# snakers4/mnasnet-pytorch

Measured on AMD Instinct MI355X. Metric: images/sec MNASNet-1.0 224^2 bf16 train step, higher is better.
Workload: dtype bf16

## Files before the change

include/mnas.h:

```cpp
#ifndef MNAS_H
#define MNAS_H
#include <stdint.h>

#ifdef __cplusplus
extern "C" {
#endif

#define MNAS_OK 0
#define MNAS_EINVAL 10001
#define MNAS_BN_ROWS 8

typedef struct MnasActIn {
    const void*  data;
    const float* scale;
    const float* shift;
} MnasActIn;

typedef struct MnasGradIn {
    const void*  g;
    const void*  y;
    const float* coef;
} MnasGradIn;

int mnas_version(void);
const char* mnas_arch(void);

typedef struct MnasConvGemm {
    int32_t mode;
    int32_t N, Hi, Wi, Ci;
    int32_t Ho, Wo, Co;
    int32_t kh, kw, stride, pad;
    int32_t nparts;
    int32_t reserved;
    MnasActIn  act;
    MnasGradIn grad;
    const void*  w;
    const float* bias;
    const void*  resid;
    void*        out;
    float*       stats;
    const void*  red_y;
    const float* red_bn;
    const float* gate;
} MnasConvGemm;
int mnas_conv_gemm_gate_ok(int N, int HW, int Ci, int Co);
int mnas_conv_gemm(const MnasConvGemm* a, void* stream);
int mnas_conv_gemm_tile_pixels(int M, int Co, int K);
int mnas_conv_gemm_parts(int mode, int M, int Ci, int Co, int taps);
int mnas_conv_img_parts(int mode, int N, int Hi, int Wi, int Ci, int Ho, int Wo, int Co, int k, int stride, int pad);
#define MNAS_ROUTE_PWX   0
#define MNAS_ROUTE_PWS   1
#define MNAS_ROUTE_PWF   2
#define MNAS_ROUTE_PWD   3
#define MNAS_ROUTE_C3R   4
#define MNAS_ROUTE_DIMG  5
#define MNAS_ROUTE_C3X   6
#define MNAS_ROUTE_IGEMM 7
int mnas_conv_gemm_route(const MnasConvGemm* a, int* out);

typedef struct MnasTconvDgrad {
    int32_t N, Ho, Wo, Co, Ci, nparts;
    const void* dy;
    const void* w;
    void* out;
    float* stats;
    const void* red_y;
    const float* red_bn;
} MnasTconvDgrad;
int mnas_tconv_dgrad(const MnasTconvDgrad* a, void* stream);
int mnas_tconv_supported(int Ho, int Wo, int Co, int Ci);
int mnas_tconv_parts(int N, int Ho, int Wo, int Co, int Ci);

typedef struct MnasConvWgrad {
    int32_t N, Hi, Wi, Ci;
    int32_t Ho, Wo, Co;
    int32_t kh, kw, stride, pad;
    int32_t nsplit;
    MnasActIn  x;
    MnasGradIn dy;
    float* partial;
} MnasConvWgrad;
int mnas_conv_wgrad(const MnasConvWgrad* a, void* stream);
int mnas_conv_wgrad_slabs(int Co, int Ci, int taps);

int mnas_wgrad_finalize(float* partial, int nsplit, int Co, int Ci, int taps,
                        float* grad, int accumulate, void* stream);

typedef struct MnasPwBwd {
    int32_t M, Ci, Co, nparts;
    MnasActIn  x;
    MnasGradIn dy;
    const void* w;
    const void* resid;
    void*  gin;
    float* wpartial;
    float* red_partial;
    const void*  red_y;
    const float* red_bn;
    const void*  w_fwd;
    const float* b_fwd;
    int32_t gin_masked;
    int32_t seg_px;
} MnasPwBwd;
int mnas_pw_bwd(const MnasPwBwd* a, void* stream);
int mnas_pw_bwd_supported(int Ci, int Co);
int mnas_pw_bwd_tile_pixels(int Ci, int Co);
int mnas_pw_bwd_slices(int Ci, int Co);
int mnas_pw_bwd_forms(int Ci, int Co);

typedef struct MnasDwFwd {
    int32_t N, H, W, C, k;
    int32_t nparts;
    MnasActIn in;
    const float* w;
    const float* bias;
    void*  out;
    float* stats;
    int32_t stride, reserved;
} MnasDwFwd;
int mnas_dw_fwd(const MnasDwFwd* a, void* stream);
int mnas_dw_geometry(int N, int H, int W, int C, int k, int which, int* out);
int mnas_dw_rows(int N, int H, int W, int C, int k, int nparts, int which);

typedef struct MnasDwBwd {
    int32_t N, H, W, C, k;
    int32_t nparts;
    MnasActIn  x;
    MnasGradIn dy;
    const float* w;
    void*  gin;
    float* wpartial;
    const float* red_bn;
    float* red_partial;
    int32_t phase;
    int32_t stride;
    int32_t g_masked, reserved;
} MnasDwBwd;
int mnas_dw_bwd(const MnasDwBwd* a, void* stream);
int mnas_dw_wgrad_finalize(float* wpartial, int nparts, int C, int k, float* grad, int accumulate,
                           void* stream);

typedef struct MnasStemFwd {
    int32_t N, H, W, Ho, Wo, Co;
    int32_t nparts;
    const float* x;
    const void*  w;
    const float* bias;
    void*  out;
    float* stats;
    const float* in_affine;
    int32_t in_u8, reserved;
} MnasStemFwd;
int mnas_stem_fwd(const MnasStemFwd* a, void* stream);
typedef struct MnasStemWgrad {
    int32_t N, H, W, Ho, Wo, Co;
    int32_t nparts;
    const float* x;
    MnasGradIn dy;
    float* partial;
    const float* in_affine;
    int32_t in_u8, reserved;
} MnasStemWgrad;
int mnas_stem_wgrad(const MnasStemWgrad* a, void* stream);
int mnas_stem_parts(int which, int N, int H, int W, int Co);
int mnas_stem_dgrad(const MnasGradIn* dy, const float* w, int N, int H, int W, int Ho, int Wo, int Co, const float* in_affine,
                    float* dx, void* stream);

int mnas_bn_fwd_finalize(const float* partial, int nparts, int C, double count,
                         const float* gamma, const float* beta,
                         float* running_mean, float* running_var, int64_t* num_batches_tracked,
                         float momentum, float eps, int training, float* bnbuf, void* stream);
int mnas_bn_bwd_reduce(const void* g, const void* y, const float* bnbuf, int64_t rows, int C,
                       int nparts, float* partial, void* stream);
int mnas_dy_materialize(const MnasGradIn* d, int64_t rows, int C, void* out_bf16, void* stream);
int mnas_bn_bwd_finalize(const float* partial, int nparts, int C, double count,
                         float* bnbuf, float* dgamma, float* dbeta, int accumulate, void* stream);

typedef struct MnasPostWgrad {
    float* partial;
    float* grad;
    int32_t nsplit, Co, Ci, taps, dw, level;
} MnasPostWgrad;
typedef struct MnasBwdPost {
    const float* bn_partial;
    float* bnbuf;
    float* dgamma;
    float* dbeta;
    double count;
    int32_t bn_nparts, bn_C;
    MnasPostWgrad w1, w2;
} MnasBwdPost;
int mnas_bwd_post(const MnasBwdPost* p, void* stream);

typedef struct MnasBnFrozenDesc {
    const float* gamma;
    const float* beta;
    const float* running_mean;
    const float* running_var;
    float*  bnbuf;
    int32_t C;
    float   eps;
} MnasBnFrozenDesc;
int mnas_bn_frozen_tables(const MnasBnFrozenDesc* descs, int n, void* stream);
int mnas_bn_bwd_finalize_frozen(const float* partial, int nparts, int C, const float* bnbuf, float* dgamma, float* dbeta,
                                float* dbias, int accumulate, void* stream);
typedef struct MnasBwdPostFrozen {
    const float* bn_partial;
    const float* bnbuf;
    float* dgamma;
    float* dbeta;
    double count;
// ... 284 lines not shown
```

mnasnet_pytorch_amd/_lib.py:

```python
from __future__ import annotations

import ctypes as C
import os

import torch

_HERE = os.path.dirname(os.path.abspath(__file__))
ABI_VERSION = 8
LIB_PATH = os.environ.get("MNAS_LIB_PATH") or os.path.join(_HERE, "csrc", "libmnas_hip.so")

c_void_p, c_int, c_float, c_double, c_int64 = C.c_void_p, C.c_int, C.c_float, C.c_double, C.c_int64


class MnasActIn(C.Structure):
    _fields_ = [("data", c_void_p), ("scale", c_void_p), ("shift", c_void_p)]


class MnasGradIn(C.Structure):
    _fields_ = [("g", c_void_p), ("y", c_void_p), ("coef", c_void_p)]


class MnasConvGemm(C.Structure):
    _fields_ = [("mode", C.c_int32), ("N", C.c_int32), ("Hi", C.c_int32), ("Wi", C.c_int32), ("Ci", C.c_int32),
                ("Ho", C.c_int32), ("Wo", C.c_int32), ("Co", C.c_int32), ("kh", C.c_int32), ("kw", C.c_int32),
# ... 160 lines not shown
    OP_BWD_POST: (("bn_nparts", "bn_C") + _post("w1") + _post("w2"), ("count",),
                  ("bn_partial", "bnbuf", "dgamma", "dbeta", "w1.partial", "w1.grad", "w2.partial", "w2.grad")),
    OP_BWD_POST_FROZEN: (("bn_nparts", "bn_C") + _post("w1") + _post("w2"), ("count",),
                         ("bn_partial", "bnbuf", "dgamma", "dbeta", "w1.partial", "w1.grad", "w2.partial", "w2.grad", "dbias")),
    OP_BN_BWD_FINALIZE_FROZEN: (("nparts", "C", "accumulate"), (), ("partial", "bnbuf", "dgamma", "dbeta", "dbias")),
    OP_BN_FROZEN_BATCH: (("n",), (), ("descs",)),
    OP_TCONV_DGRAD: (("N", "Ho", "Wo", "Co", "Ci", "nparts"), (), ("dy", "w", "out", "stats", "red_y", "red_bn")),
    OP_HEAD_LINEAR: (("N", "I", "O", "relu", "accumulate", "which"), (),
                     ("x", "w", "b", "y", "dz", "dw", "db", "dx", "relu_mask")),
    OP_SE_SCALE: (("N", "HW", "C"), (), _act("a") + ("u", "out")),
    OP_SE_BWD_REDUCE: (("N", "HW", "C"), (), ("gs",) + _act("a") + ("u", "du", "scratch")),
    OP_SE_BWD_APPLY: (("N", "HW", "C"), (), ("gs", "u", "dz", "out", "red_y", "red_bn", "red_partial")),
    OP_SE_GATE: (("N", "C"), (), ("u", "gate")),
    OP_SE_PROJ_FIN: (("N", "kseg", "Co", "Ci", "accumulate"), (), ("wpartial", "u", "w", "grad", "du")),
    OP_SE_FC_FWD: (("N", "E", "R"), (), ("z", "w1", "b1", "w2", "b2", "hb", "u", "gate")),
    OP_SE_FC_BWD: (("N", "E", "R", "accumulate"), (), ("du", "z", "hb", "w1", "w2", "dh", "dz", "dw1", "db1", "dw2", "db2")),
}
OP_STREAM_SLOT = 14
_SLOT = {}
_GROUP = {}
for _opc, _kinds in OP_SLOTS.items():
    _SLOT[_opc], _GROUP[_opc] = {}, {}
    for _kind, _names in zip("idp", _kinds):
        for _k, _name in enumerate(_names):
            if _name is None:
                continue
            if _name in _SLOT[_opc] or (_kind == "i" and _k >= OP_STREAM_SLOT):
                raise ValueError("OP_SLOTS[%d]: bad slot %s" % (_opc, _name))
            _SLOT[_opc][_name] = (_kind, _k)
            if "." in _name:
                _GROUP[_opc].setdefault(_name.split(".")[0], []).append(_name)


def slot(opcode, name):
    return _SLOT[opcode][name][1]


def set_op(o, opcode, stream=0, **fields):
    slots, oi, od, op = _SLOT[opcode], o.i, o.d, o.p
    o.opcode, oi[OP_STREAM_SLOT] = opcode, stream
    for name, v in fields.items():
        where = slots.get(name)
        if where is None:
            members = _GROUP[opcode].get(name)
            if members is None:
                raise TypeError("opcode %d: unknown slot %s" % (opcode, name))
            if hasattr(v, "_asdict"):
                v = [getattr(v, m.split(".")[1]) for m in members]
            elif hasattr(v, "act_ptrs"):
                v = v.act_ptrs()
            if len(v) != len(members) or any(m in fields for m in members):
                raise TypeError("opcode %d: group %s takes %d values, once" % (opcode, name, len(members)))
            set_op(o, opcode, stream, **dict(zip(members, v)))
            continue
        kind, k = where
        if kind == "i":
            oi[k] = v
        elif kind == "d":
            od[k] = v
        else:
            op[k] = (v if v is None or type(v) is int else v.data_ptr()) or None
    return o


def op_field(o, name):
    kind, k = _SLOT[o.opcode][name]
    return getattr(o, kind)[k]


def op_ints(o):
    return tuple(int(v) for v in o.i[:len(OP_SLOTS[o.opcode][0])])


class MnasHeadLinear(C.Structure):
    _fields_ = [("N", C.c_int32), ("I", C.c_int32), ("O", C.c_int32), ("relu", C.c_int32), ("accumulate", C.c_int32),
                ("drop_p", c_float), ("seed", C.c_uint64), ("x", c_void_p), ("w", c_void_p), ("b", c_void_p),
                ("y", c_void_p), ("dz", c_void_p), ("dw", c_void_p), ("db", c_void_p), ("dx", c_void_p),
                ("relu_mask", c_void_p)]


METERS_MAX_K, METERS_NUM_I64, METERS_NUM_F64 = 4, 14, 3


class MnasMeters(C.Structure):
    _fields_ = [("steps", c_int64), ("samples", c_int64), ("loss_samples", c_int64), ("nonfinite_steps", c_int64),
                ("correct", c_int64 * 4), ("last_n", c_int64), ("last_loss_n", c_int64), ("last_correct", c_int64 * 4),
                ("loss_sum", c_double), ("last_loss", c_double), ("last_loss_sum", c_double)]


MLABEL_NUM_I64, MLABEL_NUM_F64 = 16, 9


class MnasMultiLabelMeters(C.Structure):
    _fields_ = [(n, c_int64) for n in ("steps", "samples", "nonfinite_steps", "loss_n", "dice_n", "f1_n", "tp", "fp", "fn", "last_n",
                                       "last_loss_n", "last_dice_n", "last_f1_n", "last_tp", "last_fp", "last_fn")] + \
               [(n, c_double) for n in ("loss_sum", "dice_sum", "f1_sum", "last_loss", "last_dice", "last_f1", "last_loss_sum",
                                        "last_dice_sum", "last_f1_sum")]


GRADNORM_MAX_PARTS = 1024


class MnasGradStats(C.Structure):
    _fields_ = [("last_norm", c_float), ("last_coef", c_float), ("steps", c_int64), ("clipped_steps", c_int64),
                ("skipped_steps", c_int64)]


class MnasOptExtra(C.Structure):
    _fields_ = [("partial", c_void_p), ("nparts", C.c_int32), ("max_norm", c_float), ("skip_nonfinite", C.c_int32),
                ("ema", c_void_p), ("ema_decay", c_float), ("stats", c_void_p), ("update_stats", C.c_int32)]


SYMBOLS = {
    "mnas_conv_img_parts": (c_int, [c_int] * 11),
    "mnas_stem_parts": (c_int, [c_int, c_int, c_int, c_int, c_int]),
    "mnas_head_linear_fwd": (c_int, [C.POINTER(MnasHeadLinear), c_void_p]),
    "mnas_head_linear_bwd_w": (c_int, [C.POINTER(MnasHeadLinear), c_void_p]),
    "mnas_head_linear_bwd_x": (c_int, [C.POINTER(MnasHeadLinear), c_void_p]),
    "mnas_head_dropout_mask": (c_int, [c_void_p, c_int64, c_float, C.c_uint64, c_void_p]),
    "mnas_head_cross_entropy": (c_int, [c_void_p, c_void_p, c_int, c_int, c_int64, c_void_p, c_void_p, c_void_p, c_void_p,
                                        c_void_p]),
    "mnas_head_cross_entropy_metrics": (c_int, [c_void_p, c_void_p, c_int, c_int, c_int64, c_void_p, c_void_p, c_void_p, c_void_p,
                                                C.POINTER(c_int), c_int, c_void_p, c_void_p, c_void_p]),
    "mnas_head_metrics": (c_int, [c_void_p, c_void_p, c_int, c_int, C.POINTER(c_int), c_int, c_void_p, c_void_p, c_void_p,
                                  c_void_p]),
    "mnas_head_cross_entropy_soft": (c_int, [c_void_p, c_void_p, c_void_p, c_void_p, c_float, c_int, c_int, c_int64, c_void_p,
                                             c_void_p, c_void_p, c_void_p, C.POINTER(c_int), c_int, c_void_p, c_void_p, c_void_p]),
    "mnas_mlabel_scratch_bytes": (c_int64, [c_int]),
    "mnas_mlabel_bce": (c_int, [c_void_p, c_void_p, c_void_p, c_int, c_int, c_int, c_float, c_float, c_void_p, c_void_p, c_void_p,
                                c_void_p, c_int64, c_int64, c_int64, c_void_p]),
    "mnas_mlabel_metrics": (c_int, [c_void_p, c_void_p, c_int, c_int, c_void_p, c_void_p, c_void_p, c_int64, c_int64, c_int64,
                                    c_void_p]),
    "mnas_mlabel_hard_dice": (c_int, [c_void_p, c_void_p, c_int, c_int, c_float, c_int, c_void_p, c_void_p, c_void_p]),
    "mnas_se_scale": (c_int, [C.POINTER(MnasActIn), c_void_p, c_int, c_int, c_int, c_void_p, c_void_p]),
    "mnas_se_bwd_reduce": (c_int, [c_void_p, C.POINTER(MnasActIn), c_void_p, c_int, c_int, c_int, c_void_p, c_void_p, c_void_p]),
    "mnas_se_scratch_bytes": (c_int64, [c_int, c_int, c_int]),
    "mnas_se_bwd_apply": (c_int, [c_void_p, c_void_p, c_void_p, c_int, c_int, c_int, c_void_p, c_void_p, c_void_p, c_void_p, c_void_p]),
    "mnas_se_bwd_apply_cols": (c_int, [c_int, c_int, c_int]),
    "mnas_se_gate": (c_int, [c_void_p, c_int, c_int, c_void_p, c_void_p]),
    "mnas_se_proj_finalize": (c_int, [c_void_p, c_int, c_int, c_int, c_int, c_void_p, c_void_p, c_void_p, c_int, c_void_p, c_void_p]),
    "mnas_stem_dgrad": (c_int, [c_void_p, c_void_p] + [c_int] * 6 + [c_void_p] * 3),
    "mnas_se_fc_supported": (c_int, [c_int, c_int]),
    "mnas_se_fc_fwd": (c_int, [c_void_p] * 5 + [c_int] * 3 + [c_void_p] * 4),
    "mnas_se_fc_bwd": (c_int, [c_void_p] * 5 + [c_int] * 3 + [c_void_p] * 6 + [c_int, c_void_p]),
    "mnas_conv_gemm_gate_ok": (c_int, [c_int, c_int, c_int, c_int]),
    "mnas_graph_create": (c_int, [C.POINTER(MnasOp), c_int, C.POINTER(c_void_p), c_int, C.POINTER(c_void_p), C.POINTER(c_int)]),
    "mnas_graph_launch": (c_int, [c_void_p, c_void_p]),
    "mnas_graph_destroy": (c_int, [c_void_p]),
    "mnas_version": (c_int, []),
    "mnas_arch": (C.c_char_p, []),
    "mnas_workspace_bytes": (c_int64, [c_int, c_int, c_int, c_int]),
    "mnas_conv_gemm": (c_int, [C.POINTER(MnasConvGemm), c_void_p]),
    "mnas_conv_gemm_route": (c_int, [C.POINTER(MnasConvGemm), C.POINTER(c_int)]),
    "mnas_conv_gemm_tile_pixels": (c_int, [c_int, c_int, c_int]),
    "mnas_conv_gemm_parts": (c_int, [c_int, c_int, c_int, c_int, c_int]),
    "mnas_conv_wgrad": (c_int, [C.POINTER(MnasConvWgrad), c_void_p]),
    "mnas_conv_wgrad_slabs": (c_int, [c_int, c_int, c_int]),
    "mnas_wgrad_finalize": (c_int, [c_void_p, c_int, c_int, c_int, c_int, c_void_p, c_int, c_void_p]),
    "mnas_pw_bwd": (c_int, [C.POINTER(MnasPwBwd), c_void_p]),
    "mnas_pw_bwd_supported": (c_int, [c_int, c_int]),
    "mnas_pw_bwd_forms": (c_int, [c_int, c_int]),
    "mnas_pw_bwd_tile_pixels": (c_int, [c_int, c_int]),
    "mnas_pw_bwd_slices": (c_int, [c_int, c_int]),
    "mnas_dw_fwd": (c_int, [C.POINTER(MnasDwFwd), c_void_p]),
    "mnas_dw_bwd": (c_int, [C.POINTER(MnasDwBwd), c_void_p]),
    "mnas_dw_rows": (c_int, [c_int, c_int, c_int, c_int, c_int, c_int, c_int]),
    "mnas_dw_geometry": (c_int, [c_int, c_int, c_int, c_int, c_int, c_int, C.POINTER(c_int)]),
    "mnas_dw_wgrad_finalize": (c_int, [c_void_p, c_int, c_int, c_int, c_void_p, c_int, c_void_p]),
    "mnas_stem_fwd": (c_int, [C.POINTER(MnasStemFwd), c_void_p]),
    "mnas_stem_wgrad": (c_int, [C.POINTER(MnasStemWgrad), c_void_p]),
    "mnas_bn_fwd_finalize": (c_int, [c_void_p, c_int, c_int, c_double, c_void_p, c_void_p, c_void_p, c_void_p,
                                     c_void_p, c_float, c_float, c_int, c_void_p, c_void_p]),
    "mnas_bn_bwd_reduce": (c_int, [c_void_p, c_void_p, c_void_p, c_int64, c_int, c_int, c_void_p, c_void_p]),
    "mnas_tconv_dgrad": (c_int, [C.POINTER(MnasTconvDgrad), c_void_p]),
    "mnas_tconv_supported": (c_int, [c_int, c_int, c_int, c_int]),
    "mnas_tconv_parts": (c_int, [c_int, c_int, c_int, c_int, c_int]),
    "mnas_bwd_post": (c_int, [C.POINTER(MnasBwdPost), c_void_p]),
    "mnas_bwd_post_frozen": (c_int, [C.POINTER(MnasBwdPostFrozen), c_void_p]),
    "mnas_bn_bwd_finalize_frozen": (c_int, [c_void_p, c_int, c_int, c_void_p, c_void_p, c_void_p, c_void_p, c_int, c_void_p]),
    "mnas_bn_frozen_tables": (c_int, [c_void_p, c_int, c_void_p]),
    "mnas_dy_materialize": (c_int, [C.POINTER(MnasGradIn), c_int64, c_int, c_void_p, c_void_p]),
    "mnas_bn_bwd_finalize": (c_int, [c_void_p, c_int, c_int, c_double, c_void_p, c_void_p, c_void_p, c_int, c_void_p]),
    "mnas_add_act": (c_int, [C.POINTER(MnasActIn), C.POINTER(MnasActIn), c_int64, c_int, c_void_p, c_void_p, c_int,
                             c_void_p]),
    "mnas_pool_act": (c_int, [C.POINTER(MnasActIn), c_int, c_int, c_int, c_void_p, c_void_p]),
    "mnas_pool_bwd": (c_int, [c_void_p, c_int, c_int, c_int, c_void_p, c_void_p]),
    "mnas_nchw_f32_to_nhwc_bf16": (c_int, [c_void_p, c_void_p, c_int, c_int, c_int, c_void_p]),
    "mnas_pack_weights": (c_int, [c_void_p, c_int, c_int, c_int, c_int, c_int, c_void_p, c_void_p]),
    "mnas_pack_weights_batch": (c_int, [c_void_p, c_int, c_void_p]),
    "mnas_packed_bytes": (c_int64, [c_int, c_int, c_int, c_int, c_int]),
    "mnas_adam_step": (c_int, [c_void_p, c_void_p, c_void_p, c_void_p, c_int64, c_float, c_float, c_float, c_float,
                               c_float, c_int, c_float, c_void_p]),
    "mnas_rmsprop_step": (c_int, [c_void_p, c_void_p, c_void_p, c_void_p, c_int64, c_float, c_float, c_float, c_float, c_float,
                                  c_float, c_void_p]),
    "mnas_sgd_step": (c_int, [c_void_p, c_void_p, c_void_p, c_int64, c_float, c_float, c_float, c_float, c_int, c_int, c_float,
                              c_void_p]),
    "mnas_grad_sqnorm": (c_int, [c_void_p, c_int64, c_float, c_void_p, c_int, C.POINTER(c_int), c_void_p]),
    "mnas_adam_step_ex": (c_int, [c_void_p, c_void_p, c_void_p, c_void_p, c_int64, c_float, c_float, c_float, c_float,
                                  c_float, c_int, c_float, C.POINTER(MnasOptExtra), c_void_p]),
    "mnas_rmsprop_step_ex": (c_int, [c_void_p, c_void_p, c_void_p, c_void_p, c_int64, c_float, c_float, c_float, c_float, c_float,
                                     c_float, C.POINTER(MnasOptExtra), c_void_p]),
    "mnas_sgd_step_ex": (c_int, [c_void_p, c_void_p, c_void_p, c_int64, c_float, c_float, c_float, c_float, c_int, c_int, c_float,
                                 C.POINTER(MnasOptExtra), c_void_p]),
    "mnas_run_ops": (c_int, [C.POINTER(MnasOp), c_int, c_void_p, C.POINTER(c_int)]),
    "mnas_run_ops_multi": (c_int, [C.POINTER(MnasOp), c_int, C.POINTER(c_void_p), c_int, C.POINTER(c_int)]),
    "mnas_event_create": (c_int, [C.POINTER(c_void_p)]),
    "mnas_event_destroy": (c_int, [c_void_p]),
    "mnas_event_record": (c_int, [c_void_p, c_void_p]),
    "mnas_event_elapsed_ms": (c_int, [c_void_p, c_void_p, C.POINTER(c_float)]),
    "mnas_probe_copy": (c_int, [c_void_p, c_void_p, c_int64, c_void_p]),
    "mnas_probe_valu": (c_int, [c_void_p, c_int, c_int, c_void_p]),
    "mnas_probe_copy4": (c_int, [c_void_p, c_void_p, c_int64, c_int, c_void_p]),
    "mnas_probe_read": (c_int, [c_void_p, c_void_p, c_int64, c_int, c_void_p]),
    "mnas_probe_empty": (c_int, [c_int, c_int, c_void_p]),
    "mnas_img_xform_check": (c_int, [C.POINTER(MnasImgXform), c_int, c_int, c_int, c_int64]),
    "mnas_img_xform": (c_int, [c_void_p, c_int, c_int, c_int, c_void_p, c_int64, c_void_p, c_void_p]),
    "mnas_img_color_check": (c_int, [C.POINTER(MnasImgColor), c_int, c_int, c_int]),
    "mnas_img_color_workspace_bytes": (c_int64, [c_int, c_int, c_int]),
    "mnas_img_color": (c_int, [c_void_p, c_int, c_int, c_int, c_int, c_void_p, c_int, c_void_p, c_void_p, c_void_p]),
    "mnas_img_mix_check": (c_int, [C.POINTER(MnasImgMix), c_int, c_int, c_int]),
    "mnas_img_mix": (c_int, [c_void_p, c_int, c_int, c_int, c_void_p, c_void_p, c_void_p]),
}

_lib = None


def load():
    global _lib
    if _lib is not None:
        return _lib
    if not os.path.exists(LIB_PATH):
        raise RuntimeError(
            "libmnas_hip.so not built (%s): run `make -C mnasnet_pytorch_amd/csrc` or __graft_entry__.build(). "
            "There is no CPU / eager fallback for the MNASNet hot path." % LIB_PATH)
    lib = C.CDLL(LIB_PATH)
    for name, (res, args) in SYMBOLS.items():
        fn = getattr(lib, name)
        fn.restype = res
        fn.argtypes = args
    if lib.mnas_version() != ABI_VERSION:
        raise RuntimeError("libmnas_hip.so ABI version %d != %d (stale build: run make -C mnasnet_pytorch_amd/csrc)" % (lib.mnas_version(), ABI_VERSION))
    _lib = lib
    return lib


def check(rc, what="mnas call"):
    if rc != 0:
        raise RuntimeError("%s failed with code %d" % (what, rc))


def cur_stream():
    return torch.cuda.current_stream().cuda_stream


def ptr(t):
    return 0 if t is None else t.data_ptr()
```

mnasnet_pytorch_amd/csrc/mnas_gemm.hip:

```cpp
#include "mnas_common.h"

struct IgemmArgs {
    int M, Hi, Wi, Ci, Ho, Wo, Co;
    int kh, kw, stride, pad;
    int Ktot, Kpad, kch, taps, is_pw, co_pad16;
    int s2, Mc, tpc;
    MnasActIn act;
    MnasGradIn grad;
    const uint16_t* w;
    const float* bias;
    const void* resid;
    void* out;
    float* stats;
    const void* red_y;
    const float* red_bn;
    int nt;
    float rcp_hw, rcp_wo, rcp_ci;
    const float* gate;
};

template <int MODE, int NT, int PT, int KCH, bool PIPE, bool PAR2, bool GATE = false>
__global__ __launch_bounds__(256) void k_igemm(IgemmArgs a) {
    static_assert(!GATE || (MODE == 0 && !PAR2), "the gate is an act-on-load extension of the 1x1 forward");
    extern __shared__ __attribute__((aligned(16))) unsigned char smem[];
// ... 426 lines not shown
    if (a.s2) a.tpc = (a.Mc + 64 * PT - 1) / (64 * PT);
    const int ntiles = a.s2 ? 4 * a.tpc : (a.M + 64 * PT - 1) / (64 * PT);
    const int nkc = (a.Kpad + a.kch - 1) / a.kch;
    const int phases = nkc * ((ntiles + nparts - 1) / nparts);
    const bool s2 = a.taps > 1 && a.stride == 2;
    bool pipe;
    if (MODE == 0) pipe = phases >= 4 && !(s2 && PT == 2) && !(NT >= 6 && PT == 2);
    else pipe = phases >= 2 && nkc > 1 && !s2;
    if constexpr (PT == 1 && (NT == 2 || NT == 3 || NT == 4 || NT == 6)) {
        if (a.kch == 128) return launch_igemm_k<MODE, NT, PT, 128>(a, nparts, nblocks, pipe, stream);
    }
    return a.kch >= 64 ? launch_igemm_k<MODE, NT, PT, 64>(a, nparts, nblocks, pipe, stream)
                       : launch_igemm_k<MODE, NT, PT, 32>(a, nparts, nblocks, pipe, stream);
}

static void igemm_tiling(int Co, int Kpad, int M, int* nt_out, int* nblocks_out, int* pt_out) {
    const int tiles = (Co + 15) / 16;
    int best_nt = 1, best_waste = 1 << 30, best_blocks = 1 << 30;
    if (tiles <= 8) {
        static const int opts1[] = {1, 2, 3, 4, 6, 8};
        for (int nt : opts1) if (nt >= tiles) { best_nt = nt; best_blocks = 1; break; }
    } else {
        static const int opts_small_k[3] = {4, 3, 0}, opts_large_k[3] = {6, 4, 3};
        for (int nt : (Kpad >= 512 ? opts_large_k : opts_small_k)) {
            if (nt == 0) continue;
            const int blocks = (tiles + nt - 1) / nt;
            const int waste = blocks * nt - tiles;
            if (waste < best_waste || (waste == best_waste && blocks < best_blocks)) {
                best_nt = nt; best_waste = waste; best_blocks = blocks;
            }
        }
    }
    *nt_out = best_nt;
    *nblocks_out = best_blocks;
    *pt_out = ((int64_t)M * best_blocks >= (int64_t)128 * 1024) ? 2 : 1;
}

extern "C" int mnas_conv_gemm_tile_pixels(int M, int Co, int K) {
    if (M < 1 || Co < 1 || K < 1) return -1;
    int nt, nblocks, pt;
    igemm_tiling(Co, (K + 31) / 32 * 32, M, &nt, &nblocks, &pt);
    return 64 * pt;
}

extern "C" int mnas_conv_gemm_parts(int mode, int M, int Ci, int Co, int taps) {
    if (mode == 0 && taps == 1) {
        const int p = mnas_pwx_parts(M, Ci, Co);
        if (p > 0) return p;
    }
    if (taps == 1) {
        const int p = mnas_pws_parts(mode, M, Ci, Co);
        if (p > 0) return p;
    }
    if (mode == 0 && taps == 1 && mnas_pwf_enabled()) return mnas_pwf_parts(M, Ci, Co);
    if (mode == 1 && taps == 1 && mnas_pwd_enabled()) return mnas_pwd_parts(M, Ci, Co);
    return -1;
}

extern "C" int mnas_conv_gemm_gate_ok(int N, int HW, int Ci, int Co) {
    if (N < 1 || HW < 1 || (Ci & 7) || (Co & 7) || Ci < 8 || Co < 8) return 0;
    const int M = N * HW;
    if (mnas_pws_parts(0, M, Ci, Co) > 0) return mnas_pws_gate_ok(M, Ci, Co);
    int nt, nblocks, pt;
    igemm_tiling(Co, (Ci + 31) / 32 * 32, M, &nt, &nblocks, &pt);
    return (nt <= 3 && nblocks == 1 && !(pt == 1 && Ci >= 256) && HW >= 64 * pt) ? 1 : 0;
}

static int conv_gemm_plan(const MnasConvGemm* c, IgemmArgs* ap, int* nt_out, int* nblocks_out, int* pt_out) {
    if (!c || (c->mode != 0 && c->mode != 1)) return -MNAS_EINVAL;
    if ((c->Ci & 7) || (c->Co & 7) || c->nparts < 1 || c->nparts > 65535) return -MNAS_EINVAL;
    IgemmArgs& a = *ap;
    a.M = c->N * c->Ho * c->Wo;
    a.Hi = c->Hi; a.Wi = c->Wi; a.Ci = c->Ci; a.Ho = c->Ho; a.Wo = c->Wo; a.Co = c->Co;
    a.kh = c->kh; a.kw = c->kw; a.stride = c->stride; a.pad = c->pad;
    a.taps = c->kh * c->kw;
    a.Ktot = a.taps * c->Ci;
    a.Kpad = (a.Ktot + 31) / 32 * 32;
    a.kch = a.Kpad >= 64 ? 64 : 32;
    a.is_pw = (a.taps == 1 && c->stride == 1 && c->pad == 0) ? 1 : 0;
    a.co_pad16 = (c->Co + 15) / 16 * 16;
    a.act = c->act; a.grad = c->grad;
    a.w = (const uint16_t*)c->w; a.bias = c->bias; a.resid = c->resid; a.out = c->out; a.stats = c->stats;
    a.red_y = (c->mode == 1) ? c->red_y : nullptr; a.red_bn = c->red_bn;
    a.nt = (mnas_nt_mask() & (c->mode == 1 ? MNAS_NT_IGEMM_DGRAD : MNAS_NT_IGEMM_FWD)) ? 1 : 0;
    a.gate = c->gate;
    if (a.gate && (c->mode != 0 || !a.is_pw || !c->act.scale || c->resid)) return -MNAS_EINVAL;
    {
        const int s2f = (c->mode == 1 && c->kh == 3 && c->kw == 3 && c->stride == 2 && c->pad == 1 && !(c->Ho & 1) && !(c->Wo & 1));
        const int wd = s2f ? c->Wo / 2 : c->Wo, hwd = s2f ? (c->Ho / 2) * wd : c->Ho * c->Wo;
        const bool small = (int64_t)a.M < (1 << 24);
        a.rcp_hw = small ? 1.0f / (float)hwd : 0.f;
        a.rcp_wo = small ? 1.0f / (float)wd : 0.f;
        a.rcp_ci = 1.0f / (float)c->Ci;
    }
    a.s2 = (c->mode == 1 && c->kh == 3 && c->kw == 3 && c->stride == 2 && c->pad == 1 && !(c->Ho & 1) && !(c->Wo & 1)) ? 1 : 0;
    a.Mc = c->N * (c->Ho / 2) * (c->Wo / 2);
    a.tpc = 0;
    if (a.red_y && (!a.red_bn || !a.stats)) return -MNAS_EINVAL;
    if (a.taps != 1 && c->Ci > 1024) return -MNAS_EINVAL;
    if (a.taps == 1 && !a.is_pw) return -MNAS_EINVAL;
    if (c->mode == 0 && !c->act.data) return -MNAS_EINVAL;
    if (c->mode == 1 && (!c->grad.g || (!c->grad.y) != (!c->grad.coef))) return -MNAS_EINVAL;
    if (c->mode == 0 && a.is_pw && !c->resid && !c->gate && mnas_pwx_parts(a.M, c->Ci, c->Co) > 0)
        return MNAS_ROUTE_PWX;
    if (a.is_pw && (c->mode == 1 || !c->resid) && mnas_pws_parts(c->mode, a.M, c->Ci, c->Co) > 0 && mnas_pws_accepts(c))
        return MNAS_ROUTE_PWS;
    if (c->mode == 0 && a.is_pw && !c->resid && !c->gate && mnas_pwf_enabled() && mnas_pwf_parts(a.M, c->Ci, c->Co) > 0)
        return MNAS_ROUTE_PWF;
    if (c->mode == 1 && a.is_pw && !c->resid && !c->bias && mnas_pwd_enabled() && mnas_pwd_parts(a.M, c->Ci, c->Co) > 0)
        return MNAS_ROUTE_PWD;

    if (a.taps == 9 && !c->resid && !(c->mode == 1 && c->grad.y) &&
        mnas_c3r_parts(c->mode, c->N, c->Hi, c->Wi, c->Ci, c->Ho, c->Wo, c->Co, c->kh, c->kw, c->stride, c->pad) > 0)
        return MNAS_ROUTE_C3R;
    if (a.taps == 9 && !(c->mode == 0 && c->resid) && !(c->mode == 1 && (c->grad.y || c->resid)) &&
        mnas_dimg_parts(c->mode, c->N, c->Hi, c->Wi, c->Ci, c->Ho, c->Wo, c->Co, c->kh, c->kw, c->stride, c->pad) > 0)
        return MNAS_ROUTE_DIMG;

    if (c->mode == 0 && a.taps == 9 && !c->resid && !c->gate &&
        mnas_c3x_ok(c->N, c->Hi, c->Wi, c->Ci, c->Ho, c->Wo, c->Co, c->kh, c->kw, c->stride, c->pad))
        return MNAS_ROUTE_C3X;

    igemm_tiling(c->Co, a.Kpad, a.M, nt_out, nblocks_out, pt_out);
    const int best_nt = *nt_out, pt = *pt_out;
    if (pt == 1 && a.Kpad >= 256 && (best_nt == 2 || best_nt == 3 || best_nt == 6 || (best_nt == 4 && mnas_diag_env("MNAS_IG_K128_NT4", 1)))) a.kch = 128;
    return MNAS_ROUTE_IGEMM;
}

extern "C" int mnas_conv_gemm_route(const MnasConvGemm* c, int* out) {
    IgemmArgs a;
    int nt = 0, nblocks = 0, pt = 0;
    const int route = conv_gemm_plan(c, &a, &nt, &nblocks, &pt);
    if (out) {
        out[0] = out[1] = out[2] = out[3] = 0;
        if (route == MNAS_ROUTE_IGEMM) { out[0] = nt; out[1] = pt; out[2] = a.kch; out[3] = a.s2; }
    }
    return route;
}

extern "C" int mnas_conv_gemm(const MnasConvGemm* c, void* stream) {
    IgemmArgs a;
    int best_nt = 0, nblocks = 0, pt = 0;
    switch (conv_gemm_plan(c, &a, &best_nt, &nblocks, &pt)) {
        case MNAS_ROUTE_PWX: return mnas_pwx_forward(c, stream);
        case MNAS_ROUTE_PWS: return mnas_pws_run(c, stream);
        case MNAS_ROUTE_PWF: return mnas_pwf_forward(c, stream);
        case MNAS_ROUTE_PWD: return mnas_pwd_dgrad(c, stream);
        case MNAS_ROUTE_C3R: return mnas_c3r_run(c, stream);
        case MNAS_ROUTE_DIMG: return mnas_dimg_run(c, stream);
        case MNAS_ROUTE_C3X: return mnas_c3x_run(c, stream);
        case MNAS_ROUTE_IGEMM: break;
        default: return MNAS_EINVAL;
    }
    hipStream_t s = (hipStream_t)stream;
#define MNAS_IG(MODE_, NT_) \
    if (c->mode == MODE_ && best_nt == NT_) return pt == 2 ? launch_igemm<MODE_, NT_, 2>(a, c->nparts, nblocks, s) \
                                                           : launch_igemm<MODE_, NT_, 1>(a, c->nparts, nblocks, s);
    MNAS_IG(0, 1) MNAS_IG(0, 2) MNAS_IG(0, 3) MNAS_IG(0, 4) MNAS_IG(0, 6) MNAS_IG(0, 8)
    MNAS_IG(1, 1) MNAS_IG(1, 2) MNAS_IG(1, 3) MNAS_IG(1, 4) MNAS_IG(1, 6) MNAS_IG(1, 8)
#undef MNAS_IG
    return MNAS_EINVAL;
}

extern "C" int mnas_stem_fwd(const MnasStemFwd* c, void* stream) {
    if (!c || (c->Co & 7) || c->Co > 128 || c->nparts < 1) return MNAS_EINVAL;
    {
        const int rc = mnas_stem_fwd_band(c, stream);
        if (rc != MNAS_EINVAL) return rc;
    }
    if (c->in_affine || c->in_u8) return MNAS_EINVAL;
    IgemmArgs a;
    a.M = c->N * c->Ho * c->Wo;
    a.Hi = c->H; a.Wi = c->W; a.Ci = 27; a.Ho = c->Ho; a.Wo = c->Wo; a.Co = c->Co;
    a.kh = 3; a.kw = 3; a.stride = 2; a.pad = 1;
    a.taps = 1; a.Ktot = 27; a.Kpad = 32; a.kch = 32; a.is_pw = 0;
    a.co_pad16 = (c->Co + 15) / 16 * 16;
    a.act.data = c->x; a.act.scale = nullptr; a.act.shift = nullptr;
    a.grad.g = nullptr; a.grad.y = nullptr; a.grad.coef = nullptr;
    a.w = (const uint16_t*)c->w; a.bias = c->bias; a.resid = nullptr; a.out = c->out; a.stats = c->stats;
    a.red_y = nullptr; a.red_bn = nullptr; a.gate = nullptr;
    a.nt = (mnas_nt_mask() & MNAS_NT_STEM) ? 1 : 0;
    a.rcp_hw = (int64_t)a.M < (1 << 24) ? 1.0f / (float)(c->Ho * c->Wo) : 0.f;
    a.rcp_wo = (int64_t)a.M < (1 << 24) ? 1.0f / (float)c->Wo : 0.f;
    a.rcp_ci = 0.f;
    a.s2 = 0; a.Mc = 0; a.tpc = 0;
    const int tiles = (c->Co + 15) / 16;
    hipStream_t s = (hipStream_t)stream;
    if (tiles == 1) return launch_igemm_k<2, 1, 2, 32>(a, c->nparts, 1, true, s);
    if (tiles == 2) return launch_igemm_k<2, 2, 2, 32>(a, c->nparts, 1, true, s);
    if (tiles <= 4) return launch_igemm_k<2, 4, 2, 32>(a, c->nparts, 1, true, s);
    return launch_igemm_k<2, 8, 2, 32>(a, c->nparts, 1, true, s);
}
```

Measured before the change: 25970.

## Add specialized narrow pointwise forward kernel with prefetched loads for small Co

Adds a dedicated 1x1 forward conv kernel for narrow output channels (Co<=32, Ci<=96). It keeps the weights in registers, streams input through buffer loads prefetched one or two groups ahead, applies BN-on-load, runs MFMA, and writes through a per-wave LDS stage while accumulating BN stats. It is routed only for large M and the specific shapes (72->24, 32->16). Its aim is to cut the overhead of the generic igemm on these memory-bound projection layers. In exchange it adds another code path to maintain, and the routing is tuned to those shapes.

```diff
diff --git a/include/mnas.h b/include/mnas.h
--- a/include/mnas.h
+++ b/include/mnas.h
@@ -57,6 +57,9 @@
 #define MNAS_ROUTE_C3X   6
 #define MNAS_ROUTE_IGEMM 7
 int mnas_conv_gemm_route(const MnasConvGemm* a, int* out);
+int mnas_pwn_routed(int M, int Ci, int Co);
+int mnas_pwn_forward(const MnasConvGemm* a, void* stream);
+int mnas_pwn_waves(int Ci, int Co);
 
 typedef struct MnasTconvDgrad {
     int32_t N, Ho, Wo, Co, Ci, nparts;
diff --git a/mnasnet_pytorch_amd/_lib.py b/mnasnet_pytorch_amd/_lib.py
--- a/mnasnet_pytorch_amd/_lib.py
+++ b/mnasnet_pytorch_amd/_lib.py
@@ -336,6 +336,9 @@
     "mnas_workspace_bytes": (c_int64, [c_int, c_int, c_int, c_int]),
     "mnas_conv_gemm": (c_int, [C.POINTER(MnasConvGemm), c_void_p]),
     "mnas_conv_gemm_route": (c_int, [C.POINTER(MnasConvGemm), C.POINTER(c_int)]),
+    "mnas_pwn_routed": (c_int, [c_int, c_int, c_int]),
+    "mnas_pwn_forward": (c_int, [C.POINTER(MnasConvGemm), c_void_p]),
+    "mnas_pwn_waves": (c_int, [c_int, c_int]),
     "mnas_conv_gemm_tile_pixels": (c_int, [c_int, c_int, c_int]),
     "mnas_conv_gemm_parts": (c_int, [c_int, c_int, c_int, c_int, c_int]),
     "mnas_conv_wgrad": (c_int, [C.POINTER(MnasConvWgrad), c_void_p]),
diff --git a/mnasnet_pytorch_amd/csrc/mnas_gemm.hip b/mnasnet_pytorch_amd/csrc/mnas_gemm.hip
--- a/mnasnet_pytorch_amd/csrc/mnas_gemm.hip
+++ b/mnasnet_pytorch_amd/csrc/mnas_gemm.hip
@@ -602,6 +602,8 @@
         case MNAS_ROUTE_IGEMM: break;
         default: return MNAS_EINVAL;
     }
+    if (c->mode == 0 && a.is_pw && !c->resid && !c->gate && c->Hi == c->Ho && c->Wi == c->Wo && mnas_pwn_routed(a.M, c->Ci, c->Co))
+        return mnas_pwn_forward(c, stream);
     hipStream_t s = (hipStream_t)stream;
 #define MNAS_IG(MODE_, NT_) \
     if (c->mode == MODE_ && best_nt == NT_) return pt == 2 ? launch_igemm<MODE_, NT_, 2>(a, c->nparts, nblocks, s) \
diff --git a/mnasnet_pytorch_amd/csrc/mnas_pwn.hip b/mnasnet_pytorch_amd/csrc/mnas_pwn.hip
--- /dev/null
+++ b/mnasnet_pytorch_amd/csrc/mnas_pwn.hip
@@ -0,0 +1,201 @@
+#include "mnas_common.h"
+
+struct PwnArgs {
+    int M, Ci, Co;
+    int co_pad16;
+    MnasActIn act;
+    const uint16_t* w;
+    const float* bias;
+    void* out;
+    float* stats;
+};
+
+#define PWN_OOB 0x80000000u
+
+template <int TPW, int KS, int PT, int D, bool NT>
+__global__ __launch_bounds__(256) void k_pwn(PwnArgs a) {
+    constexpr int NW = 4;
+    static_assert(TPW <= 2, "one store pass: 16 pixels x Co / 8 chunks <= 64 lanes");
+    extern __shared__ __attribute__((aligned(16))) unsigned char smem[];
+    constexpr int NTH = 64 * NW, NB = TPW * 16, SP = NB + 8, Kpad = KS * 32;
+    float* lds_coef = (float*)smem;
+    float* lds_red = lds_coef + 2 * Kpad;
+    uint16_t* stage = (uint16_t*)(lds_red + NW * 2 * NB);
+    const int tid = threadIdx.x, lane = tid & 63;
+    const int wave = __builtin_amdgcn_readfirstlane(tid >> 6);
+    const int l15 = lane & 15, lg = lane >> 4;
+    const bool has_coef = a.act.scale != nullptr;
+    const __amdgpu_buffer_rsrc_t rs_in = __builtin_amdgcn_make_buffer_rsrc((void*)a.act.data, 0, a.M * a.Ci * 2, 0x00020000);
+    const __amdgpu_buffer_rsrc_t rs_out = __builtin_amdgcn_make_buffer_rsrc(a.out, 0, a.M * a.Co * 2, 0x00020000);
+
+    uint16_t* st = stage + wave * 16 * SP;
+    const int ntiles = (a.M + 64 * PT - 1) / (64 * PT);
+    auto gidx = [&](int s) { return ((int)blockIdx.x + (s / PT) * (int)gridDim.x) * (NW * PT) + wave * PT + (s % PT); };
+    u32x4_t v[D][KS];
+    auto issue = [&](u32x4_t (&dst)[KS], int gi) {
+        const unsigned m = (unsigned)gi * 16u + l15;
+#pragma unroll
+        for (int ks = 0; ks < KS; ++ks) {
+            const unsigned k = ks * 32 + lg * 8;
+            unsigned off = (m < (unsigned)a.M && k < (unsigned)a.Ci) ? (m * a.Ci + k) * 2u : PWN_OOB;
+            asm volatile("" : "+v"(off));
+            dst[ks] = __builtin_amdgcn_raw_buffer_load_b128(rs_in, off, 0, 0);
+        }
+    };
+    auto prologue = [&]() {
+#pragma unroll
+        for (int d = 0; d < D; ++d) issue(v[d], gidx(d));
+    };
+    if (MNAS_EARLY) prologue();
+    bf16x8_t wf[TPW][KS];
+#pragma unroll
+    for (int t = 0; t < TPW; ++t)
+#pragma unroll
+        for (int ks = 0; ks < KS; ++ks) {
+            const int row = t * 16 + l15;
+            uint4 x = make_uint4(0, 0, 0, 0);
+            if (row < a.co_pad16) x = *(const uint4*)(a.w + (size_t)row * Kpad + ks * 32 + lg * 8);
+            wf[t][ks] = *(const bf16x8_t*)&x;
+        }
+    mnas_fill_table(lds_coef, 2 * Kpad, tid, NTH, [&](int i) {
+        const int r = i / Kpad, c = i - r * Kpad;
+        return (has_coef && c < a.Ci) ? (r == 0 ? a.act.scale[c] : a.act.shift[c]) : 0.f;
+    });
+    float bias_r[TPW][4], s1[TPW][4], s2[TPW][4];
+#pragma unroll
+    for (int t = 0; t < TPW; ++t)
+#pragma unroll
+        for (int r = 0; r < 4; ++r) {
+            const int co = t * 16 + lg * 4 + r;
+            bias_r[t][r] = (a.bias && co < a.Co) ? a.bias[co] : 0.f;
+            s1[t][r] = 0.f; s2[t][r] = 0.f;
+        }
+    const int cpp = a.Co >> 3;
+    const int spx = lane / cpp, sch = lane - spx * cpp;
+    const uint16_t* st_rd = st + (spx & 15) * SP + sch * 8;
+#pragma unroll
+    for (int t = 0; t < TPW; ++t) {
+#pragma unroll
+        for (int ks = 0; ks < KS; ++ks) asm volatile("" :: "v"(wf[t][ks]));
+#pragma unroll
+        for (int r = 0; r < 4; ++r) asm volatile("" :: "v"(bias_r[t][r]));
+    }
+    __syncthreads();
+    if (!MNAS_EARLY) prologue();
+
+    auto group = [&](u32x4_t (&vin)[KS], int gi, int gnext) {
+        const int m0 = gi * 16;
+        const bool mok = m0 + l15 < a.M;
+        bf16x8_t bf[KS];
+#pragma unroll
+        for (int ks = 0; ks < KS; ++ks) {
+            const int k = ks * 32 + lg * 8;
+            uint4 x = make_uint4(vin[ks].x, vin[ks].y, vin[ks].z, vin[ks].w);
+            if (has_coef) {
+                float s[8], t[8];
+                *(float4*)&s[0] = *(const float4*)(lds_coef + k); *(float4*)&s[4] = *(const float4*)(lds_coef + k + 4);
+                *(float4*)&t[0] = *(const float4*)(lds_coef + Kpad + k); *(float4*)&t[4] = *(const float4*)(lds_coef + Kpad + k + 4);
+                x = act8(x, s, t);
+            }
+            bf[ks] = *(const bf16x8_t*)&x;
+        }
+        issue(vin, gnext);
+#pragma unroll
+        for (int t = 0; t < TPW; ++t) {
+            f32x4_t acc = (f32x4_t){0.f, 0.f, 0.f, 0.f};
+#pragma unroll
+            for (int ks = 0; ks < KS; ++ks) acc = __builtin_amdgcn_mfma_f32_16x16x32_bf16(wf[t][ks], bf[ks], acc, 0, 0, 0);
+            const mnas_f2 a0 = {acc[0] + bias_r[t][0], acc[1] + bias_r[t][1]}, a1 = {acc[2] + bias_r[t][2], acc[3] + bias_r[t][3]};
+            if (mok) {
+                mnas_stat2(a0, &s1[t][0], &s2[t][0]);
+                mnas_stat2(a1, &s1[t][2], &s2[t][2]);
+            }
+            uint2 pk;
+            pk.x = pack_bf16(a0.x, a0.y);
+            pk.y = pack_bf16(a1.x, a1.y);
+            *(uint2*)(st + l15 * SP + t * 16 + lg * 4) = pk;
+        }
+        __builtin_amdgcn_wave_barrier();
+        const uint4 o = *(const uint4*)st_rd;
+        unsigned ooff = (spx < 16 && m0 + spx < a.M) ? ((unsigned)m0 * a.Co + lane * 8) * 2u : PWN_OOB;
+        asm volatile("" : "+v"(ooff));
+        __builtin_amdgcn_raw_buffer_store_b128((u32x4_t){o.x, o.y, o.z, o.w}, rs_out, ooff, 0, NT ? 2 : 0);
+        __builtin_amdgcn_wave_barrier();
+    };
+    constexpr int U = D > PT ? D : PT;
+    for (int s = 0; (int)blockIdx.x + (s / PT) * (int)gridDim.x < ntiles; s += U) {
+#pragma unroll
+        for (int i = 0; i < U; ++i) group(v[i % D], gidx(s + i), gidx(s + i + D));
+    }
+
+    if (a.stats) mnas_stats_store<TPW>(s1, s2, lds_red, 0, a.Co, a.stats, tid, wave, l15, lg);
+}
+
+struct PwnPlan { int tpw, ks, pt, depth; size_t lds; };
+
+MNAS_SWITCH(mnas_pwn_mode, mnas_diag_env("MNAS_PWN", -1))
+
+static bool pwn_plan(int M, int Ci, int Co, PwnPlan* p) {
+    if ((Ci & 7) || (Co & 7) || Ci < 8 || Co < 8 || M < 1) return false;
+    if (Co > 32 || Ci > 96 || Co >= Ci) return false;
+    if ((int64_t)M * Ci * 2 >= ((int64_t)1 << 31)) return false;
+    p->tpw = (Co + 15) / 16;
+    p->ks = (Ci + 31) / 32;
+    p->pt = mnas_conv_gemm_tile_pixels(M, Co, Ci) / 64;
+    if (p->pt != 1 && p->pt != 2) return false;
+    p->depth = p->ks == 3 ? 2 : 1;
+    {
+        const int d = mnas_diag_env("MNAS_PWN_DEPTH", 0);
+        if (d == 1 || d == 2) p->depth = d;
+    }
+    const int NB = p->tpw * 16;
+    p->lds = (size_t)(2 * p->ks * 32 + 4 * 2 * NB) * 4 + (size_t)4 * 16 * (NB + 8) * 2;
+    return true;
+}
+
+extern "C" int mnas_pwn_waves(int Ci, int Co) {
+    PwnPlan p;
+    return pwn_plan(16, Ci, Co, &p) ? 4 : -1;
+}
+
+extern "C" int mnas_pwn_routed(int M, int Ci, int Co) {
+    PwnPlan p;
+    if (!pwn_plan(M, Ci, Co, &p)) return 0;
+    const int mode = mnas_pwn_mode();
+    if (mode >= 0) return mode ? 1 : 0;
+    if (M < 800000) return 0;
+    return ((Ci == 72 && Co == 24) || (Ci == 32 && Co == 16)) ? 1 : 0;
+}
+
+extern "C" int mnas_pwn_forward(const MnasConvGemm* c, void* stream) {
+    PwnPlan p;
+    if (!c || c->mode != 0 || c->kh != 1 || c->kw != 1 || c->stride != 1 || c->pad != 0) return MNAS_EINVAL;
+    if (c->Hi != c->Ho || c->Wi != c->Wo || c->N < 1 || c->Ho < 1 || c->Wo < 1) return MNAS_EINVAL;
+    if ((int64_t)c->N * c->Ho * c->Wo > ((int64_t)1 << 27)) return MNAS_EINVAL;
+    if (c->nparts < 1 || c->nparts > 65535 || c->resid || c->gate || !c->act.data || !c->w || !c->out) return MNAS_EINVAL;
+    if ((c->act.scale == nullptr) != (c->act.shift == nullptr)) return MNAS_EINVAL;
+    const int M = c->N * c->Ho * c->Wo;
+    if (!pwn_plan(M, c->Ci, c->Co, &p)) return MNAS_EINVAL;
+    PwnArgs a;
+    a.M = M; a.Ci = c->Ci; a.Co = c->Co;
+    a.co_pad16 = (c->Co + 15) / 16 * 16;
+    const bool nt = (mnas_nt_mask() & MNAS_NT_IGEMM_FWD) != 0;
+    a.act = c->act; a.w = (const uint16_t*)c->w; a.bias = c->bias; a.out = c->out; a.stats = c->stats;
+    hipStream_t s = (hipStream_t)stream;
+#define MNAS_PWN(T_, K_, P_, D_) \
+    if (p.tpw == T_ && p.ks == K_ && p.pt == P_ && p.depth == D_) { \
+        if (nt) hipLaunchKernelGGL((k_pwn<T_, K_, P_, D_, true>), dim3(c->nparts), dim3(256), p.lds, s, a); \
+        else hipLaunchKernelGGL((k_pwn<T_, K_, P_, D_, false>), dim3(c->nparts), dim3(256), p.lds, s, a); \
+        MNAS_CHECK_LAUNCH(); \
+        return MNAS_OK; \
+    }
+#define MNAS_PWN_SHAPES(P_, D12_, D3_) MNAS_PWN(1, 1, P_, D12_) MNAS_PWN(1, 2, P_, D12_) MNAS_PWN(1, 3, P_, D3_) \
+                                       MNAS_PWN(2, 1, P_, D12_) MNAS_PWN(2, 2, P_, D12_) MNAS_PWN(2, 3, P_, D3_)
+    MNAS_PWN_SHAPES(1, 1, 2) MNAS_PWN_SHAPES(2, 1, 2)
+#ifdef MNAS_DIAG
+    MNAS_PWN_SHAPES(1, 2, 1) MNAS_PWN_SHAPES(2, 2, 1)
+#endif
+#undef MNAS_PWN_SHAPES
+#undef MNAS_PWN
+    return MNAS_EINVAL;
+}
```

After: 26100 (median of 6 runs). Within noise of the previous version (+0.5%).
